# FelixWaiblinger/gym-pybullet-adrp

Measured on AMD Instinct MI355X. Metric: env-steps/sec (N parallel drones) at 1/2/4/8 MI355X; % HBM roofline, higher is better.
Workload: dtype f64; 1 GPU; HoverAviary Physics.PYB 240/30 Hz (8 sub-steps), 4096 envs x 1 drone per GPU, RPM actions, auto-reset; envs_per_gpu=4096, global_envs=4096, drones_per_env=1, parallelism=env-sharded dp1

## Files before the change

### gym_pybullet_adrp_amd/csrc/adrp_device.h

```cpp
#pragma once

#include <hip/hip_runtime.h>
#include <stdint.h>

namespace adrp {

__device__ __forceinline__ void store_out(float4* p, float4 v) {
#ifdef ADRP_NT_STORES
    typedef float f4v __attribute__((ext_vector_type(4)));
    const f4v w = {v.x, v.y, v.z, v.w};
    __builtin_nontemporal_store(w, reinterpret_cast<f4v*>(p));
#else
    *p = v;
#endif
}

#ifdef ADRP_RACE_TIMING
__device__ unsigned long long g_race_phase[32];
#define RACE_MARK(var) const uint64_t var = __builtin_amdgcn_s_memtime()
#define RACE_SET(var) var = __builtin_amdgcn_s_memtime()
#define RACE_ACC(i, dt) do { atomicAdd(&g_race_phase[i], (unsigned long long)(dt)); \
        atomicMax(&g_race_phase[10 + (i)], (unsigned long long)(dt)); } while (0)
constexpr int kWaveSlots = 16384;
__device__ unsigned long long g_race_wave[kWaveSlots * 8];
// ... 367 lines not shown
    if (x < 0.0f) r = 3.14159265358979323846f - r;
    return copysignf(r, y);
}
__device__ __forceinline__ double fatan2_(double y, double x) { return f64::atan2(y, x); }
__device__ __forceinline__ float fatan2_nc_(float y, float x) { return fatan2_(y, x); }
__device__ __forceinline__ double fatan2_nc_(double y, double x) { return f64::atan2_nc(y, x); }
__device__ __forceinline__ float fasin_(float s) { return fatan2_(s, __builtin_amdgcn_sqrtf((1.0f - s) * (1.0f + s))); }
__device__ __forceinline__ double fasin_(double s) { return f64::asin(s); }
__device__ __forceinline__ float fexp_(float x) { return __builtin_amdgcn_exp2f(x * 1.4426950408889634f); }
__device__ __forceinline__ double fexp_(double x) { return f64::exp(x); }

template <typename Real>
struct ChainK {
    Real k004, c100, nn_min, near1, tiny;
    Real ts[3], tc[4];
};
template <typename Real>
__device__ __forceinline__ ChainK<Real> chain_consts() {
    return ChainK<Real>{Real(0.04), Real(100), Real(1e-300), Real(1e-9), Real(0.03),
                        {Real(-0.0001984126984126984), Real(0.008333333333333333), Real(-0.16666666666666666)},
                        {Real(2.48015873015873e-05), Real(-0.001388888888888889), Real(0.041666666666666664), Real(-0.5)}};
}
__device__ __forceinline__ void pin(double& x) { asm volatile("" : "+v"(x)); }
__device__ __forceinline__ void pin(float&) {}
template <typename Real>
__device__ __forceinline__ void pin_all(ChainK<Real>& k) {
    pin(k.k004); pin(k.c100); pin(k.nn_min); pin(k.near1); pin(k.tiny);
#pragma unroll
    for (int i = 0; i < 3; ++i) pin(k.ts[i]);
#pragma unroll
    for (int i = 0; i < 4; ++i) pin(k.tc[i]);
}
__device__ __forceinline__ float hsqrt_nn_(float x, const ChainK<float>&) { return __builtin_amdgcn_sqrtf(x); }
__device__ __forceinline__ double hsqrt_nn_(double x, const ChainK<double>& k) {
    const double y = __builtin_amdgcn_rsq(__builtin_fmax(x, k.nn_min));
    double g = x * y, h = 0.5 * y;
#pragma unroll
    for (int i = 0; i < 2; ++i) {
        const double r = f64::fma_(-g, h, 0.5);
        g = f64::fma_(g, r, g);
        h = f64::fma_(h, r, h);
    }
    const double d = f64::fma_(-g, g, x);
    return f64::fma_(d, h, g);
}
__device__ __forceinline__ void expmap_sinc_cos(float x, float* sinc, float* c, const ChainK<float>&) {
    expmap_sinc_cos(x, sinc, c);
}
__device__ __forceinline__ void expmap_sinc_cos(double x, double* sinc, double* c, const ChainK<double>& k) {
    const double x2 = x * x;
    const bool tiny = __builtin_fabs(x) <= k.tiny;
    double ps = f64::fma_(k.ts[0], x2, k.ts[1]);
    ps = f64::fma_(ps, x2, k.ts[2]);
    double pc = f64::fma_(k.tc[0], x2, k.tc[1]);
    pc = f64::fma_(pc, x2, k.tc[2]);
    pc = f64::fma_(pc, x2, k.tc[3]);
    if (__builtin_expect(!__all(tiny), 0)) {
        double fs, fc;
        expmap_sinc_cos_full(x, &fs, &fc);
        *sinc = tiny ? f64::fma_(x2, ps, 1.0) : fs;
        *c = tiny ? f64::fma_(x2, pc, 1.0) : fc;
        return;
    }
    *sinc = f64::fma_(x2, ps, 1.0);
    *c = f64::fma_(x2, pc, 1.0);
}
struct AngK {
    double p[10];
    double tan8, pi4, pi2, pi;
    double lim, lo, hi;
};
__device__ __forceinline__ AngK ang_consts() {
    return AngK{{0.021428368220326288, -0.04375458729368037, 0.05699267039194693, -0.06642647883966969,
                 0.07690277001250925, -0.09090800003785938, 0.11111107550967636, -0.14285714221246087,
                 0.19999999999459742, -0.3333333333333199},
                0.41421356237309504880, 0.78539816339744830962, 1.57079632679489661923, 3.14159265358979323846,
                0.99999, 1e-150, 1e150};
}
__device__ __forceinline__ void pin_all(AngK& k) {
#pragma unroll
    for (int i = 0; i < 10; ++i) pin(k.p[i]);
    pin(k.tan8); pin(k.pi4); pin(k.pi2); pin(k.pi); pin(k.lim); pin(k.lo); pin(k.hi);
}
namespace f64 {
__device__ __forceinline__ bool atan2_lean_ok(double y, double x, const AngK& k) {
    const double s = __builtin_fabs(x) + __builtin_fabs(y);
    return s > k.lo && s < k.hi;
}
template <bool XPOS>
__device__ __forceinline__ double atan2_lean(double y, double x, const AngK& k) {
    const double ax = __builtin_fabs(x), ay = __builtin_fabs(y);
    const double mx = __builtin_fmax(ax, ay), mn = __builtin_fmin(ax, ay);
    const bool big = mn > k.tan8 * mx;
    const double num = big ? mn - mx : mn, den = big ? mn + mx : mx;
    const double t = num * rcp_nc(den);
    const double s = t * t;
    double p = k.p[0];
#pragma unroll
    for (int i = 1; i < 10; ++i) p = fma_(p, s, k.p[i]);
    double r = fma_(t * s, p, t);
    if (big) r += k.pi4;
    if (ay > ax) r = k.pi2 - r;
    if constexpr (!XPOS) {
        if (x < 0.0) r = k.pi - r;
    }
    return __builtin_copysign(r, y);
}
__device__ __forceinline__ double asin_lean(double s, const AngK& k) {
    const double x = (1.0 - s) * (1.0 + s);
    const double y = __builtin_amdgcn_rsq(x);
    double g = x * y, h = 0.5 * y;
#pragma unroll
    for (int i = 0; i < 2; ++i) {
        const double r = fma_(-g, h, 0.5);
        g = fma_(g, r, g);
        h = fma_(h, r, h);
    }
    const double d = fma_(-g, g, x);
    return atan2_lean<true>(s, fma_(d, h, g), k);
}
}

__device__ __forceinline__ float quat_inv_norm(float n2, const ChainK<float>&) { return quat_inv_norm(n2); }
__device__ __forceinline__ double quat_inv_norm(double n2, const ChainK<double>& k) {
    const bool near1 = __builtin_fabs(n2 - 1.0) <= k.near1;
    const double newton = f64::fma_(0.5, 1.0 - n2, 1.0);
    if (__builtin_expect(__all(near1), 1)) return newton;
    const double r = f64::rsq_nc(n2);
    return near1 ? newton : r;
}

__device__ __forceinline__ void clamp100_wv(V3<float>& w, V3<float>& v) {
    w = {__builtin_amdgcn_fmed3f(w.x, -100.0f, 100.0f), __builtin_amdgcn_fmed3f(w.y, -100.0f, 100.0f),
         __builtin_amdgcn_fmed3f(w.z, -100.0f, 100.0f)};
    v = {__builtin_amdgcn_fmed3f(v.x, -100.0f, 100.0f), __builtin_amdgcn_fmed3f(v.y, -100.0f, 100.0f),
         __builtin_amdgcn_fmed3f(v.z, -100.0f, 100.0f)};
}
__device__ __forceinline__ double clamp100_sel(double x) { return x < -100.0 ? -100.0 : (x > 100.0 ? 100.0 : x); }
__device__ __forceinline__ void clamp100_wv(V3<double>& w, V3<double>& v) {
    const bool big = (__builtin_fabs(w.x) > 100.0) | (__builtin_fabs(w.y) > 100.0) | (__builtin_fabs(w.z) > 100.0) |
                     (__builtin_fabs(v.x) > 100.0) | (__builtin_fabs(v.y) > 100.0) | (__builtin_fabs(v.z) > 100.0);
    if (__builtin_expect(__any(big), 0)) {
        w = {clamp100_sel(w.x), clamp100_sel(w.y), clamp100_sel(w.z)};
        v = {clamp100_sel(v.x), clamp100_sel(v.y), clamp100_sel(v.z)};
    }
}


template <typename Real>
__device__ __forceinline__ M3<Real> rot(Q4<Real> q) {
    const Real x2 = q.x + q.x, y2 = q.y + q.y, z2 = q.z + q.z;
    const Real xx = q.x * x2, yy = q.y * y2, zz = q.z * z2;
    const Real xy = q.x * y2, xz = q.x * z2, yz = q.y * z2;
    const Real wx = q.w * x2, wy = q.w * y2, wz = q.w * z2;
    return {Real(1) - (yy + zz), xy - wz, xz + wy,
            xy + wz, Real(1) - (xx + zz), yz - wx,
            xz - wy, yz + wx, Real(1) - (xx + yy)};
}
template <typename Real>
__device__ __forceinline__ V3<Real> mul(const M3<Real>& R, V3<Real> v) {
    return {R.a00 * v.x + R.a01 * v.y + R.a02 * v.z,
            R.a10 * v.x + R.a11 * v.y + R.a12 * v.z,
            R.a20 * v.x + R.a21 * v.y + R.a22 * v.z};
}
template <typename Real>
__device__ __forceinline__ V3<Real> mulT(const M3<Real>& R, V3<Real> v) {
// ... 154 lines not shown
```

### gym_pybullet_adrp_amd/csrc/hover_kernel.h

```cpp
#pragma once

#include "adrp_device.h"
#include "dslpid_core.h"

namespace adrp {

enum HoverField {
    HF_POS = 0, HF_QUAT = 3, HF_VEL = 7, HF_OMEGA = 10, HF_LAST_RPM = 13, HF_ANGV = 17,
    HF_LINK_QUAT = 20, HF_NBASE = 24,
    HF_PID = 24, HF_NPID = 9
};
enum HoverInt { HI_STEP = 0, HI_EPISODE = 1, HI_RING_HEAD = 2, HI_N = 3 };

template <typename Real>
struct HoverConst {
    int S, trunc_steps, link_lag, physics;
    Real dt, mass, inv_mass, gravity;
    Real ixx, iyy, izz, inv_ixx, inv_iyy, inv_izz;
    Real kf, km, hover_rpm;
    Real px[4], py[4], pz[4];
    Real gnd_kf, prop_r4, gnd_clip;
    Real drag[3];
    Real dyn_arm;
    Real coll_hh, coll_r, coll_zoff;
// ... 297 lines not shown
               c * q.z + k * (w.y * q.x - w.x * q.y + w.z * q.w),
               c * q.w + k * (-w.x * q.x - w.y * q.y - w.z * q.z)};
    }
    b.angv = mul(R, b.w);
}

template <typename Real>
__device__ __forceinline__ void hover_reset_draw(const HoverReset<Real>& a, uint64_t seed, uint64_t gid, uint32_t tag,
                                                 const HoverConst<Real>& C, Body<Real>& b, int32_t& sc, int32_t& ep) {
    const U4 r0 = draw(seed, gid, uint32_t(ep), tag, 0);
    const U4 r1 = draw(seed, gid, uint32_t(ep), tag, 1);
    const U4 r2 = draw(seed, gid, uint32_t(ep), tag, 2);
    const uint32_t w0[4] = {r0.a, r0.b, r0.c, r0.d}, w1[4] = {r1.a, r1.b, r1.c, r1.d},
                   w2[4] = {r2.a, r2.b, r2.c, r2.d};
    Real p[3], e_[3], v[3], om[3];
#pragma unroll
    for (int k = 0; k < 3; ++k) {
        p[k] = a.init_xyz[k] + a.n_xyz[k] * (Real(2) * u01r<Real>(w0[k]) - Real(1));
        e_[k] = a.init_rpy[k] + a.n_rpy[k] * (Real(2) * u01r<Real>(w1[k]) - Real(1));
        v[k] = a.n_vel[k] * (Real(2) * u01r<Real>(w2[k]) - Real(1));
    }
    om[0] = a.n_om[0] * (Real(2) * u01r<Real>(w0[3]) - Real(1));
    om[1] = a.n_om[1] * (Real(2) * u01r<Real>(w1[3]) - Real(1));
    om[2] = a.n_om[2] * (Real(2) * u01r<Real>(w2[3]) - Real(1));
    b.q = quat_from_euler_fast<Real>(e_[0], e_[1], e_[2]);
    b.pos = v3(p[0], p[1], p[2]);
    b.ql = b.q;
    b.vel = v3(v[0], v[1], v[2]);
    if (C.physics == ADRP_PHYS_DYN) {
        b.w = mulT(rot(b.q), v3(om[0], om[1], om[2]));
        b.angv = v3(om[0], om[1], om[2]);
    } else {
        b.w = v3(om[0], om[1], om[2]);
        b.angv = v3(Real(0), Real(0), Real(0));
    }
#pragma unroll
    for (int i = 0; i < 4; ++i) b.prev_rpm[i] = Real(0);
    sc = 0;
    ep += 1;
}
template <typename Real>
__device__ __forceinline__ void hover_reset_state(const HoverArgs<Real>& args, const HoverConst<Real>& C, int e,
                                                  Body<Real>& b, int32_t& sc, int32_t& ep) {
    hover_reset_draw(*args.r, args.seed, uint64_t(args.env_offset + e), TAG_HOVER_RESET, C, b, sc, ep);
}

template <typename Real>
__device__ __forceinline__ Real euler_roll_u(Q4<Real> q) {
    if (__builtin_expect(__any(fabs_(euler_sarg(q)) >= Real(0.99999)), 0)) return euler_xyz_fast(q).x;
    const EulerArgs<Real> a = euler_args(q);
    return fatan2_(a.y0, a.x0);
}
template <typename Real>
__device__ __forceinline__ Real euler_pitch_u(Q4<Real> q) {
    const Real sarg = euler_sarg(q);
    if (__builtin_expect(__any(fabs_(sarg) >= Real(0.99999)), 0)) return euler_xyz_fast(q).y;
    return fasin_(sarg);
}
template <typename Real>
__device__ __forceinline__ Real euler_yaw_u(Q4<Real> q) {
    if (__builtin_expect(__any(fabs_(euler_sarg(q)) >= Real(0.99999)), 0)) return euler_xyz_fast(q).z;
    const EulerArgs<Real> a = euler_args(q);
    return fatan2_(a.y2, a.x2);
}

__device__ __forceinline__ double euler_roll_lean(Q4<double> q, const AngK& k) {
    const EulerArgs<double> a = euler_args(q);
    const bool ok = fabs_(a.sarg) < k.lim && f64::atan2_lean_ok(a.y0, a.x0, k);
    if (__builtin_expect(__any(!ok), 0)) return euler_roll_u(q);
    return f64::atan2_lean<false>(a.y0, a.x0, k);
}
__device__ __forceinline__ double euler_pitch_lean(Q4<double> q, const AngK& k) {
    const double sarg = euler_sarg(q);
    if (__builtin_expect(__any(!(fabs_(sarg) < k.lim)), 0)) return euler_pitch_u(q);
    return f64::asin_lean(sarg, k);
}
__device__ __forceinline__ double euler_yaw_lean(Q4<double> q, const AngK& k) {
    const EulerArgs<double> a = euler_args(q);
    const bool ok = fabs_(a.sarg) < k.lim && f64::atan2_lean_ok(a.y2, a.x2, k);
    if (__builtin_expect(__any(!ok), 0)) return euler_yaw_u(q);
    return f64::atan2_lean<false>(a.y2, a.x2, k);
}

template <typename Real>
__device__ __forceinline__ Real euler_axis_u(Q4<Real> q, int ax) {
    const EulerArgs<Real> a = euler_args(q);
    const Real sarg = a.sarg;
    if (__builtin_expect(__any(fabs_(sarg) >= Real(0.99999)), 0)) {
        const V3<Real> r = euler_xyz_fast(q);
        return ax == 0 ? r.x : (ax == 1 ? r.y : r.z);
    }
    const Real y0 = a.y0, x0 = a.x0, y2 = a.y2, x2 = a.x2;
    Real x1;
    if constexpr (sizeof(Real) == 8) x1 = f64::sqrt((1.0 - sarg) * (1.0 + sarg));
    else x1 = __builtin_amdgcn_sqrtf((1.0f - sarg) * (1.0f + sarg));
    const Real yy = ax == 0 ? y0 : (ax == 1 ? sarg : y2), xx = ax == 0 ? x0 : (ax == 1 ? x1 : x2);
    return fatan2_(yy, xx);
}
__device__ __forceinline__ float readlane_r(float v, int l) {
    return __int_as_float(__builtin_amdgcn_readlane(__float_as_int(v), l));
}
__device__ __forceinline__ double readlane_r(double v, int l) {
    return __hiloint2double(__builtin_amdgcn_readlane(__double2hiint(v), l), __builtin_amdgcn_readlane(__double2loint(v), l));
}
template <typename Real>
__device__ __forceinline__ V3<Real> hover_obs12_split(const HoverConst<Real>& a, const Body<Real>& b, float o[12]) {
    const int l = int(threadIdx.x) & 63;
    const Real ang = euler_axis_u(b.q, l < 2 ? l : 2);
    const V3<Real> rpy = v3(readlane_r(ang, 0), readlane_r(ang, 1), readlane_r(ang, 2));
    const V3<Real> w = a.physics == ADRP_PHYS_DYN ? b.angv : b.w;
    o[0] = float(b.pos.x); o[1] = float(b.pos.y); o[2] = float(b.pos.z);
    o[3] = float(rpy.x);   o[4] = float(rpy.y);   o[5] = float(rpy.z);
    o[6] = float(b.vel.x); o[7] = float(b.vel.y); o[8] = float(b.vel.z);
    o[9] = float(w.x);     o[10] = float(w.y);    o[11] = float(w.z);
    return rpy;
}

template <typename Real>
__device__ __forceinline__ V3<Real> hover_obs12(const HoverConst<Real>& a, const Body<Real>& b, float o[12]) {
    const V3<Real> rpy = euler_xyz_fast_u(b.q);
    const V3<Real> w = a.physics == ADRP_PHYS_DYN ? b.angv : b.w;
    o[0] = float(b.pos.x); o[1] = float(b.pos.y); o[2] = float(b.pos.z);
    o[3] = float(rpy.x);   o[4] = float(rpy.y);   o[5] = float(rpy.z);
    o[6] = float(b.vel.x); o[7] = float(b.vel.y); o[8] = float(b.vel.z);
    o[9] = float(w.x);     o[10] = float(w.y);    o[11] = float(w.z);
    return rpy;
}

template <int A, int B>
__device__ __forceinline__ void write_row(float* row, const float o12[12], const float (&ring)[B][A], int head1) {
    if constexpr (A == 4) {
        float4* r4 = reinterpret_cast<float4*>(row);
        r4[0] = make_float4(o12[0], o12[1], o12[2], o12[3]);
        r4[1] = make_float4(o12[4], o12[5], o12[6], o12[7]);
        r4[2] = make_float4(o12[8], o12[9], o12[10], o12[11]);
#pragma unroll
        for (int p = 0; p < B; ++p) {
            int k = p - head1;
            k += k < 0 ? B : 0;
            r4[3 + k] = make_float4(ring[p][0], ring[p][1], ring[p][2], ring[p][3]);
        }
    } else {
#pragma unroll
        for (int k = 0; k < 12; ++k) row[k] = o12[k];
#pragma unroll
        for (int p = 0; p < B; ++p) {
            int k = p - head1;
            k += k < 0 ? B : 0;
#pragma unroll
            for (int j = 0; j < A; ++j) row[12 + k * A + j] = ring[p][j];
        }
    }
}

template <int A>
__device__ __forceinline__ void write_row_generic(float* __restrict__ row, const float o12[12],
                                                  const float* __restrict__ ring, int B, int E, int e, int head1,
                                                  const float act[A], bool act_is_newest) {
#pragma unroll
    for (int k = 0; k < 12; ++k) row[k] = o12[k];
    constexpr int CH = 8;
    int slot = head1;
    for (int k0 = 0; k0 < B; k0 += CH) {
        float v[CH][A];
#pragma unroll
        for (int c = 0; c < CH; ++c) {
// ... 197 lines not shown
struct NoExtForce {};
template <typename Real, int PH, int SC, bool DRAG, typename Ext>
__device__ __forceinline__ bool pyb_chain(const HoverConst<Real>& C, Body<Real>& b, const Real rpm_in[4], bool lag,
                                          Ext ext, V3<Real>* wb_out = nullptr, Real* vxy = nullptr) {
    constexpr bool EXT = !__is_same(Ext, NoExtForce);
    const Real rpm[4] = {rpm_in[0], rpm_in[1], rpm_in[2], rpm_in[3]};
    Real sum_f = 0, t2 = 0;
    V3<Real> P = v3(Real(0), Real(0), Real(0));
#pragma unroll
    for (int i = 0; i < 4; ++i) {
        const Real r2 = rpm[i] * rpm[i];
        const Real f = r2 * C.kf;
        sum_f += f;
        const bool pz0 = __builtin_constant_p(C.pz[i]) && C.pz[i] == Real(0);
        const Real fx = f * C.px[i], fy = f * C.py[i], fz = f * C.pz[i];
        P = v3(P.x + fx, P.y + fy, pz0 ? P.z : P.z + fz);
        t2 += (i & 1) ? -r2 : r2;
    }
    const Real tau_z = t2 * C.km;
    ChainK<Real> K = chain_consts<Real>();
    HoverConst<Real> Cp = C;
    if constexpr (sizeof(Real) == 8) {
        pin_all(K);
        pin(Cp.dt); pin(Cp.mass); pin(Cp.gravity); pin(Cp.inv_mass); pin(Cp.ang_max);
        pin(Cp.ixx); pin(Cp.iyy); pin(Cp.izz); pin(Cp.inv_ixx); pin(Cp.inv_iyy); pin(Cp.inv_izz);
        pin(Cp.coll_hh); pin(Cp.coll_r); pin(Cp.coll_zoff);
    }
    Chain<Real> st{};
    {
        const M3<Real> R = rot_fm(b.q);
        const M3<Real> Rs = lag ? rot_fm(b.ql) : R;
        st.wb = mulT(R, b.w);
        st.zc = col2(R);
        st.zs = col2(Rs);
        st.m3 = lag ? mulT(R, st.zs) : v3(Real(0), Real(0), Real(1));
        if constexpr (DRAG) {
            st.R = R;
            st.Rs = Rs;
        }
    }
    st.wn = hsqrt_nn_(dot(b.w, b.w), K);
    st.dti = v3(Cp.dt * Cp.inv_ixx, Cp.dt * Cp.inv_iyy, Cp.dt * Cp.inv_izz);
    bool touched = false;
    auto substep = [&](int s) {
        if constexpr (EXT) touched |= pyb_substep<Real, PH, true>(Cp, b, st, rpm, sum_f, P, tau_z, K, ext(b, st));
        else touched |= pyb_substep<Real, PH>(Cp, b, st, rpm, sum_f, P, tau_z, K, V3<Real>{}, vxy ? vxy + 2 * s : nullptr);
#pragma unroll
        for (int i = 0; i < 4; ++i) b.prev_rpm[i] = rpm[i];
    };
    if constexpr (SC > 0) {
#pragma unroll
        for (int s = 0; s < SC; ++s) substep(s);
    } else {
        for (int s = 0; s < C.S; ++s) substep(s);
    }
    if (wb_out) *wb_out = st.wb;
    else b.w = mul(rot_fm(b.q), st.wb);
    return touched;
}

constexpr int kRowF4 = 18;

template <int A, int B>
__device__ __forceinline__ void stage_row(float4* lds_row, const float o12[12], const float (&ring)[B][A], int head1) {
    lds_row[0] = make_float4(o12[0], o12[1], o12[2], o12[3]);
    lds_row[1] = make_float4(o12[4], o12[5], o12[6], o12[7]);
    lds_row[2] = make_float4(o12[8], o12[9], o12[10], o12[11]);
#pragma unroll
    for (int p = 0; p < B; ++p) {
        int k = p - head1;
        k += k < 0 ? B : 0;
        lds_row[3 + k] = make_float4(ring[p][0], ring[p][1], ring[p][2], ring[p][3]);
    }
}

template <typename Real, int PH, int A, int B, int SC, bool STG = false, int CTL = 0, bool HELP = false, int SYS = 0,
          int FO = 2>
__device__ __forceinline__ void hover_step_body(const HoverArgs<Real>& a, const HoverConst<Real>& C,
                                                const float* pre = nullptr) {
    constexpr int BR = B > 0 ? B : 1;
    constexpr bool DRAG = (PH == ADRP_PHYS_PYB_DRAG || PH == ADRP_PHYS_PYB_GND_DRAG_DW);
    constexpr bool DYN = (PH == ADRP_PHYS_DYN);
    static_assert(!HELP || STG, "the reset helper wave pairs with the staged (all lanes live) kernel");
    __shared__ Real rs_body[HELP ? kResetFields * kStepBlock : 1];
    __shared__ float rs_obs[HELP ? 12 * kStepBlock : 1];
    __shared__ float4 rows[STG ? kStepBlock * kRowF4 : 1];
    constexpr bool ANG = HELP && angle_helpers<Real>();
    __shared__ Real ang_q[ANG ? 4 * kStepBlock : 1];
    __shared__ Real ang_r[ANG ? kStepBlock : 1];
    __shared__ Real ang_p[ANG ? kStepBlock : 1];
    __shared__ float ang_y[ANG ? kStepBlock : 1];
    constexpr int kWaves = HELP ? 1 + help_waves<Real>() : 1;
    constexpr auto cb = [](int w) { return w == 0 ? 0 : (w >= kWaves ? kRowF4 : (kWaves == 2 ? kRowF4 / 2 : 5 * w - 2)); };
    constexpr bool TROWS = ANG;
    constexpr int kSplitCols = 5, kSplitRows = 12;
    static_assert(!TROWS || (cb(2) - cb(1) == kSplitCols && cb(4) - cb(3) == kSplitCols && cb(1) == 3 &&
                             kSplitCols * kSplitRows <= kStepBlock), "terminal rows: 3 + 3 x 5 columns");
    __shared__ int done_cnt[1];
    __shared__ uint8_t done_list[TROWS ? kStepBlock : 1];
    [[maybe_unused]] auto helper_tail = [&](int tl, int wv) {
        const int cnt_v = done_cnt[0];
        const int sub = tl / kSplitCols, c = cb(wv) + tl - kSplitCols * sub;
        const int row0 = done_list[sub] & (kStepBlock - 1);
        float4* dst = reinterpret_cast<float4*>(a.obs) + size_t(blockIdx.x) * kStepBlock * kRowF4;
        float4 o[kSplitCols];
#pragma unroll
        for (int j = 0; j < kSplitCols; ++j) o[j] = rows[tl + kStepBlock * (cb(wv) + j)];
        const float4 t0 = rows[row0 * kRowF4 + c];
#pragma unroll
        for (int j = 0; j < kSplitCols; ++j) store_out(dst + tl + kStepBlock * (cb(wv) + j), o[j]);
        const int cnt = __builtin_amdgcn_readfirstlane(cnt_v);
        const bool mine = tl < kSplitCols * kSplitRows;
        float4* tb = reinterpret_cast<float4*>(a.tobs) + size_t(blockIdx.x) * kStepBlock * kRowF4;
        if (mine && sub < cnt) tb[row0 * kRowF4 + c] = t0;
        for (int base = kSplitRows; base < cnt && base < kStepBlock; base += kSplitRows) {
            const int n = base + sub;
            if (mine && n < cnt) {
                const int row = done_list[n] & (kStepBlock - 1);
                tb[row * kRowF4 + c] = rows[row * kRowF4 + c];
            }
        }
    };
    if constexpr (HELP) {
        if (ANG && threadIdx.x >= 2 * kStepBlock) {
            const int tl = threadIdx.x & (kStepBlock - 1), wv = threadIdx.x / kStepBlock;
            AngK ak = ang_consts();
            pin_all(ak);
            __syncthreads();
            const Q4<Real> q = {ang_q[tl], ang_q[kStepBlock + tl], ang_q[2 * kStepBlock + tl], ang_q[3 * kStepBlock + tl]};
            if constexpr (ANG) {
                if (wv == 2) ang_p[tl] = euler_pitch_lean(q, ak);
                else ang_y[tl] = float(euler_yaw_lean(q, ak));
            }
            __syncthreads();
            __syncthreads();
            if constexpr (TROWS) {
                helper_tail(tl, wv);
                return;
            }
            float4* dst = reinterpret_cast<float4*>(a.obs) + size_t(blockIdx.x) * kStepBlock * kRowF4;
            for (int k = cb(wv); k < cb(wv + 1); ++k) store_out(dst + tl + kStepBlock * k, rows[tl + kStepBlock * k]);
            return;
        }
        if (threadIdx.x >= kStepBlock) {
            const int tl = threadIdx.x - kStepBlock;
            const int he = blockIdx.x * kStepBlock + tl;
            const int E = a.E;
            const float4 av = reinterpret_cast<const float4*>(a.act)[he];
            float rg[BR][4];
#pragma unroll
            for (int p = 0; p < B; ++p) {
                const float4 v = reinterpret_cast<const float4*>(a.ring)[size_t(p) * E + he];
                rg[p][0] = v.x; rg[p][1] = v.y; rg[p][2] = v.z; rg[p][3] = v.w;
            }
            const int32_t head = a.ist[HI_RING_HEAD * E + he];
            int32_t hsc = 0, hep = a.ist[HI_EPISODE * E + he];
            Body<Real> rb;
            hover_reset_state(a, C, he, rb, hsc, hep);
            float o[12];
            hover_obs12(C, rb, o);
            const Real v[kResetFields] = {rb.pos.x, rb.pos.y, rb.pos.z, rb.q.x, rb.q.y, rb.q.z, rb.q.w,
                                          rb.vel.x, rb.vel.y, rb.vel.z, rb.w.x, rb.w.y, rb.w.z,
                                          rb.angv.x, rb.angv.y, rb.angv.z};
#pragma unroll
            for (int k = 0; k < kResetFields; ++k) rs_body[k * kStepBlock + tl] = v[k];
#pragma unroll
            for (int k = 0; k < 12; ++k) rs_obs[k * kStepBlock + tl] = o[k];
            float4* my = rows + tl * kRowF4;
            const int hu = __builtin_amdgcn_readfirstlane(head);
            if (__all(head == hu)) {
                const int h1 = hu + 1 == B ? 0 : hu + 1;
#pragma unroll
                for (int p = 0; p < B; ++p) {
                    const int k = p >= h1 ? p - h1 : p - h1 + B;
                    my[3 + k] = make_float4(rg[p][0], rg[p][1], rg[p][2], rg[p][3]);
                }
                my[3 + B - 1] = av;
            } else {
                const int h1 = head + 1 == B ? 0 : head + 1;
#pragma unroll
                for (int p = 0; p < B; ++p) {
                    int k = p - h1;
                    k += k < 0 ? B : 0;
                    const bool hit = p == head;
                    my[3 + k] = make_float4(hit ? av.x : rg[p][0], hit ? av.y : rg[p][1], hit ? av.z : rg[p][2],
                                            hit ? av.w : rg[p][3]);
                }
            }
            reinterpret_cast<float4*>(a.ring)[size_t(head) * E + he] = av;
            [[maybe_unused]] AngK ak = ang_consts();
            if constexpr (ANG) pin_all(ak);
            __syncthreads();
            if constexpr (ANG) {
                const Q4<Real> q = {ang_q[tl], ang_q[kStepBlock + tl], ang_q[2 * kStepBlock + tl], ang_q[3 * kStepBlock + tl]};
                ang_r[tl] = euler_roll_lean(q, ak);
                __syncthreads();
            }
            __syncthreads();
            if constexpr (TROWS) {
                helper_tail(tl, 1);
                return;
            }
            float4* dst = reinterpret_cast<float4*>(a.obs) + size_t(blockIdx.x) * kStepBlock * kRowF4;
#pragma unroll
            for (int k = cb(1); k < cb(2); ++k) store_out(dst + tl + kStepBlock * k, rows[tl + kStepBlock * k]);
            return;
        }
    }
    const int E = a.E;
    const bool split = ADRP_PERSIST_SPLIT && !STG && !HELP && E == 1;
    const int e = split ? 0 : int(blockIdx.x) * kStepBlock + int(threadIdx.x);
    const int D = B > 0 ? 12 + B * A : a.D;
    if (e >= E) return;
    RACE_MARK(t0);
    const bool fit = FO == 2 ? field_offsets_fit<Real>(E) : FO == 1;
    const bool lag = C.link_lag && !DYN;
    const BodyOffs<Real> fo = body_offsets<Real>(E, e, lag, DRAG, DYN);
    uint32_t io[HI_N];
    field_run(uint32_t(e) * 4u, uint32_t(E) * 4u, 0, HI_N, io);
    Body<Real> b;
    int32_t sc, ep, head_ld;
    if (fit) {
        load_body_at<Real>(a.f, fo, b, lag, DRAG, DYN);
        sc = field_at(a.ist, io[HI_STEP]); ep = field_at(a.ist, io[HI_EPISODE]); head_ld = field_at(a.ist, io[HI_RING_HEAD]);
        field_form_end();
    } else {
        load_body(a, e, b, lag, DRAG, DYN);
        sc = a.ist[HI_STEP * E + e]; ep = a.ist[HI_EPISODE * E + e]; head_ld = a.ist[HI_RING_HEAD * E + e];
    }
    const int32_t head = head_ld;
    float act[A];
    if constexpr (SYS == 2) {
#pragma unroll
        for (int j = 0; j < A; ++j) act[j] = pre[j];
    } else if constexpr (SYS == 1) {
        uint32_t* sa = const_cast<uint32_t*>(reinterpret_cast<const uint32_t*>(a.act)) + size_t(e) * A;
#pragma unroll
        for (int j = 0; j < A; ++j)
            act[j] = __uint_as_float(__hip_atomic_load(sa + j, __ATOMIC_RELAXED, __HIP_MEMORY_SCOPE_SYSTEM));
    } else if constexpr (A == 4) {
        const float4 v = reinterpret_cast<const float4*>(a.act)[e];
        act[0] = v.x; act[1] = v.y; act[2] = v.z; act[3] = v.w;
    } else {
#pragma unroll
        for (int j = 0; j < A; ++j) act[j] = a.act[e * A + j];
    }
    float ring[BR][A];
#pragma unroll
    for (int p = 0; p < (HELP ? 0 : B); ++p) {
        if constexpr (A == 4) {
            const float4 v = reinterpret_cast<const float4*>(a.ring)[size_t(p) * E + e];
            ring[p][0] = v.x; ring[p][1] = v.y; ring[p][2] = v.z; ring[p][3] = v.w;
        } else {
#pragma unroll
            for (int j = 0; j < A; ++j) ring[p][j] = a.ring[(size_t(p) * E + e) * A + j];
        }
    }
    Real rpm[4];
    if constexpr (CTL != 0) {
        static_assert(A == (CTL == ADRP_ACT_PID ? 3 : CTL == ADRP_ACT_VEL ? 4 : 1), "PID action width");
        Real ctl[HF_NPID];
        uint32_t po[HF_PID + HF_NPID];
        field_run(uint32_t(e) * uint32_t(sizeof(Real)), uint32_t(E) * uint32_t(sizeof(Real)), HF_PID, HF_NPID, po);
        if (fit) {
#pragma unroll
            for (int k = 0; k < HF_NPID; ++k) ctl[k] = field_at(a.f, po[HF_PID + k]);
            field_form_end();
        } else {
#pragma unroll
            for (int k = 0; k < HF_NPID; ++k) ctl[k] = a.f[(HF_PID + k) * E + e];
        }
        dslpid_rpm<Real, CTL>(C, b, act, ctl, rpm);
        if (fit) {
#pragma unroll
            for (int k = 0; k < HF_NPID; ++k) field_last(a.f, po[HF_PID + k]) = ctl[k];
            field_form_end();
        } else {
#pragma unroll
            for (int k = 0; k < HF_NPID; ++k) a.f[(HF_PID + k) * E + e] = ctl[k];
        }
    } else {
#pragma unroll
        for (int i = 0; i < 4; ++i) rpm[i] = C.hover_rpm * Real(rpm_gain(act[A == 1 ? 0 : i]));
    }
    bool touched = false;
    V3<Real> wbf = v3(Real(0), Real(0), Real(0));
    constexpr bool LATE_XY = ANG && !DYN && SC > 0;
    Real vxy[LATE_XY ? 2 * SC : 2] = {};
#ifdef ADRP_RACE_TIMING
    __builtin_amdgcn_s_waitcnt(0);
#endif
    RACE_MARK(t1);
    if constexpr (DYN) {
        if constexpr (SC > 0) {
#pragma unroll
            for (int s = 0; s < SC; ++s) dyn_substep(C, b, rpm);
        } else {
            for (int s = 0; s < C.S; ++s) dyn_substep(C, b, rpm);
        }
    } else {
        touched = pyb_chain<Real, PH, SC, DRAG>(C, b, rpm, lag, NoExtForce{}, ANG ? &wbf : nullptr, LATE_XY ? vxy : nullptr);
    }
    RACE_MARK(t2);
    if (touched && a.contact_count && (!split || threadIdx.x == 0)) atomicAdd(a.contact_count, 1);
    if constexpr (HELP) {
    } else if constexpr (A == 4)
        reinterpret_cast<float4*>(a.ring)[size_t(head) * E + e] = make_float4(act[0], act[1], act[2], act[3]);
    else
#pragma unroll
        for (int j = 0; j < A; ++j) a.ring[(size_t(head) * E + e) * A + j] = act[j];
    const int BB = B > 0 ? B : a.B;
    const int head1 = head + 1 == BB ? 0 : head + 1;
    auto store_state = [&]() {
        if (fit) {
            store_body_at<Real>(a.f, fo, b, lag, DRAG, DYN);
            field_last(a.ist, io[HI_STEP]) = sc;
            field_last(a.ist, io[HI_EPISODE]) = ep;
            field_last(a.ist, io[HI_RING_HEAD]) = head1;
            field_form_end();
        } else {
            store_body(a, e, b, lag, DRAG, DYN);
            a.ist[HI_STEP * E + e] = sc;
            a.ist[HI_EPISODE * E + e] = ep;
            a.ist[HI_RING_HEAD * E + e] = head1;
        }
    };
    float o12[12];
    V3<Real> rpy;
    if constexpr (ANG) {
        const int tl = threadIdx.x;
        ang_q[tl] = b.q.x; ang_q[kStepBlock + tl] = b.q.y; ang_q[2 * kStepBlock + tl] = b.q.z;
        ang_q[3 * kStepBlock + tl] = b.q.w;
        __syncthreads();
        hold(b.q.x); hold(b.q.y); hold(b.q.z); hold(b.q.w);
        hold(wbf.x); hold(wbf.y); hold(wbf.z);
        hold(b.pos.x); hold(b.pos.y); hold(b.pos.z);
        if constexpr (LATE_XY) {
#pragma unroll
            for (int k = 0; k < 2 * SC; ++k) hold(vxy[k]);
#pragma unroll
            for (int s = 0; s < SC; ++s) {
                b.pos.x = fmx(C.dt, vxy[2 * s], b.pos.x);
                b.pos.y = fmx(C.dt, vxy[2 * s + 1], b.pos.y);
            }
        }
        hold(b.vel.x); hold(b.vel.y); hold(b.vel.z);
        if constexpr (!DYN) b.w = mul(rot_fm(b.q), wbf);
        const V3<Real> w = C.physics == ADRP_PHYS_DYN ? b.angv : b.w;
        o12[0] = float(b.pos.x); o12[1] = float(b.pos.y); o12[2] = float(b.pos.z);
        o12[6] = float(b.vel.x); o12[7] = float(b.vel.y); o12[8] = float(b.vel.z);
        o12[9] = float(w.x);     o12[10] = float(w.y);    o12[11] = float(w.z);
    } else if (split) {
        rpy = hover_obs12_split(C, b, o12);
    } else {
        rpy = hover_obs12(C, b, o12);
    }
    const Real dx = C.target[0] - b.pos.x, dy = C.target[1] - b.pos.y, dz = C.target[2] - b.pos.z;
    const Real d2 = dx * dx + dy * dy + dz * dz;
    const Real r = Real(2) - d2 * d2;
    a.rew[e] = float(r > Real(0) ? r : Real(0));
    const bool te = d2 < Real(1e-8);
    bool tr = fabs_(b.pos.x) > Real(1.5) || fabs_(b.pos.y) > Real(1.5) || b.pos.z > Real(2.0) || sc >= C.trunc_steps;
    if constexpr (ANG) {
        hold(b.w.x); hold(b.w.y); hold(b.w.z);
#pragma unroll
        for (int k = 0; k < 12; ++k)
            if (k < 3 || k > 5) hold(o12[k]);
        __syncthreads();
        rpy.x = ang_r[threadIdx.x];
        rpy.y = ang_p[threadIdx.x];
        o12[3] = float(rpy.x);
        o12[4] = float(rpy.y);
        o12[5] = ang_y[threadIdx.x];
    }
    tr = tr || fabs_(rpy.x) > Real(0.4) || fabs_(rpy.y) > Real(0.4);
    a.term[e] = te;
    a.trunc[e] = tr;
    sc += C.S;
    const bool done = a.autoreset && (te || tr);
    RACE_MARK(t3);
#ifdef ADRP_RACE_TIMING
    const unsigned long long dmask = __ballot(done);
    uint64_t t4 = 0;
#endif
    if constexpr (STG) {
        static_assert(A == 4 && B == 15, "staged rows: 72-float rows only");
        float4* my = rows + threadIdx.x * kRowF4;
        const int hu = __builtin_amdgcn_readfirstlane(head);
        if constexpr (HELP) {
        } else if (__all(head == hu)) {
            const int h1 = hu + 1 == B ? 0 : hu + 1;
#pragma unroll
            for (int p = 0; p < B; ++p) {
                const int k = p >= h1 ? p - h1 : p - h1 + B;
                my[3 + k] = make_float4(ring[p][0], ring[p][1], ring[p][2], ring[p][3]);
            }
            my[3 + B - 1] = make_float4(act[0], act[1], act[2], act[3]);
        } else {
#pragma unroll
            for (int p = 0; p < B; ++p) {
                const bool hit = p == head;
#pragma unroll
                for (int j = 0; j < A; ++j) ring[p][j] = hit ? act[j] : ring[p][j];
            }
            stage_row<A, B>(my, o12, ring, head1);
        }
        my[0] = make_float4(o12[0], o12[1], o12[2], o12[3]);
        my[1] = make_float4(o12[4], o12[5], o12[6], o12[7]);
        my[2] = make_float4(o12[8], o12[9], o12[10], o12[11]);
        if constexpr (HELP && !ANG) __syncthreads();
        if constexpr (TROWS) {
            const unsigned long long done_mask = __ballot(done);
            done_cnt[0] = a.tobs ? __popcll(done_mask) : 0;
            if (done && a.tobs) {
                float4* trow = reinterpret_cast<float4*>(a.tobs + size_t(e) * D);
                trow[0] = make_float4(o12[0], o12[1], o12[2], o12[3]);
                trow[1] = make_float4(o12[4], o12[5], o12[6], o12[7]);
                trow[2] = make_float4(o12[8], o12[9], o12[10], o12[11]);
                const uint32_t rank = __builtin_amdgcn_mbcnt_hi(uint32_t(done_mask >> 32), __builtin_amdgcn_mbcnt_lo(uint32_t(done_mask), 0u));
                done_list[rank] = uint8_t(threadIdx.x);
            }
        }
        if (done) {
            if (!TROWS && a.tobs) {
                float4 t[kRowF4];
#pragma unroll
                for (int k = 0; k < kRowF4; ++k) t[k] = my[k];
                float4* trow = reinterpret_cast<float4*>(a.tobs + size_t(e) * D);
#pragma unroll
                for (int k = 0; k < kRowF4; ++k) trow[k] = t[k];
            }
            if constexpr (HELP) {
                const int t = threadIdx.x;
                Real v[kResetFields];
#pragma unroll
                for (int k = 0; k < kResetFields; ++k) v[k] = rs_body[k * kStepBlock + t];
                b.pos = v3(v[0], v[1], v[2]);
                b.q = {v[3], v[4], v[5], v[6]};
                b.ql = b.q;
                b.vel = v3(v[7], v[8], v[9]);
                b.w = v3(v[10], v[11], v[12]);
                b.angv = v3(v[13], v[14], v[15]);
#pragma unroll
                for (int i = 0; i < 4; ++i) b.prev_rpm[i] = Real(0);
                sc = 0;
                ep += 1;
#pragma unroll
                for (int k = 0; k < 12; ++k) o12[k] = rs_obs[k * kStepBlock + t];
            } else {
                hover_reset_state(a, C, e, b, sc, ep);
                hover_obs12(C, b, o12);
            }
            my[0] = make_float4(o12[0], o12[1], o12[2], o12[3]);
            my[1] = make_float4(o12[4], o12[5], o12[6], o12[7]);
            my[2] = make_float4(o12[8], o12[9], o12[10], o12[11]);
        }
        RACE_SET(t4);
        store_state();
        __syncthreads();
        float4* dst = reinterpret_cast<float4*>(a.obs) + size_t(blockIdx.x) * kStepBlock * kRowF4;
        constexpr int KC = cb(1);
#pragma unroll
        for (int k = 0; k < KC; ++k) store_out(dst + threadIdx.x + kStepBlock * k, rows[threadIdx.x + kStepBlock * k]);
    } else {
#pragma unroll
        for (int p = 0; p < B; ++p) {
            const bool hit = p == head;
#pragma unroll
            for (int j = 0; j < A; ++j) ring[p][j] = hit ? act[j] : ring[p][j];
        }
        if (done) {
            if (a.tobs) {
                if constexpr (B > 0) write_row<A, B>(a.tobs + size_t(e) * D, o12, ring, head1);
                else write_row_generic<A>(a.tobs + size_t(e) * D, o12, a.ring, a.B, E, e, head1, act, true);
            }
            hover_reset_state(a, C, e, b, sc, ep);
            if (split) hover_obs12_split(C, b, o12);
            else hover_obs12(C, b, o12);
        }
        RACE_SET(t4);
        if constexpr (B > 0) write_row<A, B>(a.obs + size_t(e) * D, o12, ring, head1);
        else write_row_generic<A>(a.obs + size_t(e) * D, o12, a.ring, a.B, E, e, head1, act, true);
    }
    RACE_MARK(t5);
    if constexpr (!STG) {
        store_state();
    }
#ifdef ADRP_RACE_TIMING
    RACE_MARK(t6);
    if (threadIdx.x == 0) {
        RACE_ACC(0, t1 - t0); RACE_ACC(1, t2 - t1); RACE_ACC(2, t3 - t2); RACE_ACC(3, t4 - t3);
        RACE_ACC(4, t5 - t4); RACE_ACC(5, t6 - t5); RACE_ACC(6, t6 - t0); RACE_ACC(8, 1);
        RACE_ACC(7, __popcll(dmask));
        if (dmask) atomicAdd(&g_race_phase[9], 1ull);
    }
#endif
}

template <typename Real>
struct HoverTail {
    const HoverConst<Real>* c;
    const HoverReset<Real>* r;
    uint8_t* term;
    uint8_t* trunc;
    float* tobs;
    int32_t* contact_count;
    uint64_t seed;
    int64_t env_offset;
    int B, D, autoreset;
};

template <typename Real, int PH, int A, int B, bool DEF, bool STG = false, int CTL = 0, bool HELP = false, bool W32 = true>
__global__ void __launch_bounds__(256) hover_step_kernel(Real* f, float* ring, int32_t* ist, const float* act,
                                                         float* obs, float* rew, int E, HoverTail<Real> t) {
    HoverArgs<Real> a;
    a.c = t.c; a.r = t.r;
    a.f = f; a.ring = ring; a.ist = ist; a.act = act; a.obs = obs; a.rew = rew;
    a.term = t.term; a.trunc = t.trunc; a.tobs = t.tobs; a.mask = nullptr; a.contact_count = t.contact_count;
    a.seed = t.seed; a.env_offset = t.env_offset;
    a.E = E; a.B = t.B; a.D = t.D; a.autoreset = t.autoreset;
    if constexpr (DEF) {
        constexpr HoverConst<Real> C = cf2x_consts<Real>(PH);
        hover_step_body<Real, PH, A, B, C.S, STG, CTL, HELP, 0, W32 ? 1 : 0>(a, C);
    } else {
        hover_step_body<Real, PH, A, B, 0, STG, CTL, HELP, 0, W32 ? 1 : 0>(a, *a.c);
    }
}

template <typename Real, int A>
__global__ void __launch_bounds__(256) hover_reset_kernel(HoverArgs<Real> a) {
    const int e = blockIdx.x * blockDim.x + threadIdx.x;
    if (e >= a.E || (a.mask && !a.mask[e])) return;
    const HoverConst<Real>& C = *a.c;
    const int E = a.E;
    const bool dyn = C.physics == ADRP_PHYS_DYN;
    const bool drag = C.physics == ADRP_PHYS_PYB_DRAG || C.physics == ADRP_PHYS_PYB_GND_DRAG_DW;
    Body<Real> b;
    int32_t sc = a.ist[HI_STEP * E + e], ep = a.ist[HI_EPISODE * E + e];
    const int head = a.ist[HI_RING_HEAD * E + e];
    hover_reset_state(a, C, e, b, sc, ep);
    store_body(a, e, b, C.link_lag && !dyn, drag, dyn);
    a.ist[HI_STEP * E + e] = sc;
    a.ist[HI_EPISODE * E + e] = ep;
    float o12[12];
    hover_obs12(C, b, o12);
    const float none[A] = {};
// ... 5 lines not shown
```

Baseline: 765.8 million env-steps/s.

## Decide truncation from quaternion directly and move obs copy-out to helper waves

```diff
diff --git a/gym_pybullet_adrp_amd/csrc/adrp_device.h b/gym_pybullet_adrp_amd/csrc/adrp_device.h
--- a/gym_pybullet_adrp_amd/csrc/adrp_device.h
+++ b/gym_pybullet_adrp_amd/csrc/adrp_device.h
@@ -473,6 +473,20 @@
     for (int i = 0; i < 10; ++i) pin(k.p[i]);
     pin(k.tan8); pin(k.pi4); pin(k.pi2); pin(k.pi); pin(k.lim); pin(k.lo); pin(k.hi);
 }
+constexpr double kTruncBand = 1e-9;
+struct TruncK {
+    double s_lo, s_hi, t_lo, t_hi;
+    double lim;
+};
+__device__ __forceinline__ TruncK trunc_consts() {
+    return TruncK{0.3894183423086505 * (1.0 - kTruncBand), 0.3894183423086505 * (1.0 + kTruncBand),
+                  0.4227932187381618 * (1.0 - kTruncBand), 0.4227932187381618 * (1.0 + kTruncBand), 0.99999};
+}
+__device__ __forceinline__ void pin_s(double& x) { asm volatile("" : "+s"(x)); }
+__device__ __forceinline__ void pin_all(TruncK& k) {
+    pin_s(k.s_lo); pin_s(k.s_hi); pin_s(k.t_lo); pin_s(k.t_hi); pin_s(k.lim);
+}
+
 namespace f64 {
 __device__ __forceinline__ bool atan2_lean_ok(double y, double x, const AngK& k) {
     const double s = __builtin_fabs(x) + __builtin_fabs(y);
diff --git a/gym_pybullet_adrp_amd/csrc/hover_kernel.h b/gym_pybullet_adrp_amd/csrc/hover_kernel.h
--- a/gym_pybullet_adrp_amd/csrc/hover_kernel.h
+++ b/gym_pybullet_adrp_amd/csrc/hover_kernel.h
@@ -403,6 +403,16 @@
     return f64::atan2_lean<false>(a.y2, a.x2, k);
 }
 
+__device__ __forceinline__ bool trunc_from_quat(Q4<double> q, const TruncK& k, bool& over) {
+    const EulerArgs<double> a = euler_args(q);
+    const double as = fabs_(a.sarg), ay = fabs_(a.y0);
+    const bool p_over = as > k.s_hi, r_over = ay > k.t_hi * a.x0;
+    const bool p_sure = p_over || as < k.s_lo, r_sure = r_over || ay < k.t_lo * a.x0;
+    over = p_over || r_over;
+    return p_sure && r_sure && a.x0 > 0.0 && as < k.lim;
+}
+__device__ __forceinline__ bool trunc_from_quat(Q4<float>, const TruncK&, bool&) { return false; }
+
 template <typename Real>
 __device__ __forceinline__ Real euler_axis_u(Q4<Real> q, int ax) {
     const EulerArgs<Real> a = euler_args(q);
@@ -766,38 +776,72 @@
     constexpr bool DRAG = (PH == ADRP_PHYS_PYB_DRAG || PH == ADRP_PHYS_PYB_GND_DRAG_DW);
     constexpr bool DYN = (PH == ADRP_PHYS_DYN);
     static_assert(!HELP || STG, "the reset helper wave pairs with the staged (all lanes live) kernel");
+    constexpr bool ANG = HELP && angle_helpers<Real>();
     __shared__ Real rs_body[HELP ? kResetFields * kStepBlock : 1];
-    __shared__ float rs_obs[HELP ? 12 * kStepBlock : 1];
-    __shared__ float4 rows[STG ? kStepBlock * kRowF4 : 1];
-    constexpr bool ANG = HELP && angle_helpers<Real>();
+    __shared__ float rs_obs[HELP && !ANG ? 12 * kStepBlock : 1];
+    constexpr int kResetObs = kStepBlock * kRowF4;
+    __shared__ float4 rows[STG ? kStepBlock * kRowF4 + (ANG ? 3 * kStepBlock : 0) : 1];
     __shared__ Real ang_q[ANG ? 4 * kStepBlock : 1];
     __shared__ Real ang_r[ANG ? kStepBlock : 1];
     __shared__ Real ang_p[ANG ? kStepBlock : 1];
     __shared__ float ang_y[ANG ? kStepBlock : 1];
     constexpr int kWaves = HELP ? 1 + help_waves<Real>() : 1;
-    constexpr auto cb = [](int w) { return w == 0 ? 0 : (w >= kWaves ? kRowF4 : (kWaves == 2 ? kRowF4 / 2 : 5 * w - 2)); };
+    constexpr auto cb = [](int w) { return w == 0 ? 0 : (w >= kWaves ? kRowF4 : (kWaves == 2 ? kRowF4 / 2 : 6 * (w - 1))); };
     constexpr bool TROWS = ANG;
-    constexpr int kSplitCols = 5, kSplitRows = 12;
-    static_assert(!TROWS || (cb(2) - cb(1) == kSplitCols && cb(4) - cb(3) == kSplitCols && cb(1) == 3 &&
-                             kSplitCols * kSplitRows <= kStepBlock), "terminal rows: 3 + 3 x 5 columns");
+    constexpr int kHelpLanes = 3 * kStepBlock, kRingF4 = kRowF4 - 3;
+    constexpr int kRingPer = kStepBlock * kRingF4 / kHelpLanes;
+    constexpr int kTermRows = kHelpLanes / kRowF4;
+    static_assert(!TROWS || (kWaves == 4 && kRingPer * kHelpLanes == kStepBlock * kRingF4 && cb(1) == 0),
+                  "copy-out over three helper waves");
     __shared__ int done_cnt[1];
     __shared__ uint8_t done_list[TROWS ? kStepBlock : 1];
-    [[maybe_unused]] auto helper_tail = [&](int tl, int wv) {
+    __shared__ uint8_t done_b[TROWS ? kStepBlock : 1];
+    struct TailIdx {
+        uint32_t ring[kRingPer], kin, fix, flag, sub, tcol;
+    };
+    [[maybe_unused]] auto tail_index = [&](int tl, int wv) {
+        TailIdx t;
+        const uint32_t g = uint32_t(wv - 1) * kStepBlock + uint32_t(tl);
+#pragma unroll
+        for (int j = 0; j < kRingPer; ++j) {
+            const uint32_t n = g + kHelpLanes * uint32_t(j);
+            const uint32_t row = (n * 4370u) >> 16;
+            t.ring[j] = (row * kRowF4 + 3u + (n - kRingF4 * row)) * 16u;
+            asm volatile("" : "+v"(t.ring[j]));
+        }
+        t.flag = (g * 21846u) >> 16;
+        t.kin = (t.flag * kRowF4 + (g - 3u * t.flag)) * 16u;
+        t.fix = (kResetObs + g) * 16u;
+        t.sub = (g * 3641u) >> 16;
+        t.tcol = g - kRowF4 * t.sub;
+        asm volatile("" : "+v"(t.kin), "+v"(t.fix), "+v"(t.flag), "+v"(t.sub), "+v"(t.tcol));
+        return t;
+    };
+    [[maybe_unused]] auto helper_ring = [&](const TailIdx& ti) {
+        const char* lds = reinterpret_cast<const char*>(rows);
+        char* dst = reinterpret_cast<char*>(a.obs) + size_t(blockIdx.x) * (kStepBlock * kRowF4 * sizeof(float4));
+        float4 o[kRingPer];
+#pragma unroll
+        for (int j = 0; j < kRingPer; ++j) o[j] = *reinterpret_cast<const float4*>(lds + ti.ring[j]);
+#pragma unroll
+        for (int j = 0; j < kRingPer; ++j) store_out(reinterpret_cast<float4*>(dst + ti.ring[j]), o[j]);
+    };
+    [[maybe_unused]] auto helper_tail = [&](const TailIdx& ti) {
         const int cnt_v = done_cnt[0];
-        const int sub = tl / kSplitCols, c = cb(wv) + tl - kSplitCols * sub;
-        const int row0 = done_list[sub] & (kStepBlock - 1);
-        float4* dst = reinterpret_cast<float4*>(a.obs) + size_t(blockIdx.x) * kStepBlock * kRowF4;
-        float4 o[kSplitCols];
-#pragma unroll
-        for (int j = 0; j < kSplitCols; ++j) o[j] = rows[tl + kStepBlock * (cb(wv) + j)];
-        const float4 t0 = rows[row0 * kRowF4 + c];
-#pragma unroll
-        for (int j = 0; j < kSplitCols; ++j) store_out(dst + tl + kStepBlock * (cb(wv) + j), o[j]);
+        const int row0 = done_list[ti.sub] & (kStepBlock - 1);
+        const uint8_t fl = done_b[ti.flag];
+        const char* lds = reinterpret_cast<const char*>(rows);
+        char* dst = reinterpret_cast<char*>(a.obs) + size_t(blockIdx.x) * (kStepBlock * kRowF4 * sizeof(float4));
+        const float4 o = *reinterpret_cast<const float4*>(lds + (fl ? ti.fix : ti.kin));
+        float4 t0 = rows[row0 * kRowF4 + int(ti.tcol)];
+        hold(t0.x); hold(t0.y); hold(t0.z); hold(t0.w);
+        store_out(reinterpret_cast<float4*>(dst + ti.kin), o);
         const int cnt = __builtin_amdgcn_readfirstlane(cnt_v);
-        const bool mine = tl < kSplitCols * kSplitRows;
+        const int sub = int(ti.sub), c = int(ti.tcol);
+        const bool mine = sub < kTermRows;
         float4* tb = reinterpret_cast<float4*>(a.tobs) + size_t(blockIdx.x) * kStepBlock * kRowF4;
         if (mine && sub < cnt) tb[row0 * kRowF4 + c] = t0;
-        for (int base = kSplitRows; base < cnt && base < kStepBlock; base += kSplitRows) {
+        for (int base = kTermRows; base < cnt && base < kStepBlock; base += kTermRows) {
             const int n = base + sub;
             if (mine && n < cnt) {
                 const int row = done_list[n] & (kStepBlock - 1);
@@ -810,16 +854,26 @@
             const int tl = threadIdx.x & (kStepBlock - 1), wv = threadIdx.x / kStepBlock;
             AngK ak = ang_consts();
             pin_all(ak);
+            const TailIdx ti = tail_index(tl, wv);
             __syncthreads();
             const Q4<Real> q = {ang_q[tl], ang_q[kStepBlock + tl], ang_q[2 * kStepBlock + tl], ang_q[3 * kStepBlock + tl]};
             if constexpr (ANG) {
-                if (wv == 2) ang_p[tl] = euler_pitch_lean(q, ak);
-                else ang_y[tl] = float(euler_yaw_lean(q, ak));
-            }
+                float* rowf = reinterpret_cast<float*>(rows) + tl * (4 * kRowF4);
+                if (wv == 2) {
+                    const double p = euler_pitch_lean(q, ak);
+                    ang_p[tl] = p;
+                    rowf[4] = float(p);
+                } else {
+                    const float y = float(euler_yaw_lean(q, ak));
+                    ang_y[tl] = y;
+                    rowf[5] = y;
+                }
+            }
+            if constexpr (TROWS) helper_ring(ti);
             __syncthreads();
             __syncthreads();
             if constexpr (TROWS) {
-                helper_tail(tl, wv);
+                helper_tail(ti);
                 return;
             }
             float4* dst = reinterpret_cast<float4*>(a.obs) + size_t(blockIdx.x) * kStepBlock * kRowF4;
@@ -848,8 +902,14 @@
                                           rb.angv.x, rb.angv.y, rb.angv.z};
 #pragma unroll
             for (int k = 0; k < kResetFields; ++k) rs_body[k * kStepBlock + tl] = v[k];
-#pragma unroll
-            for (int k = 0; k < 12; ++k) rs_obs[k * kStepBlock + tl] = o[k];
+            if constexpr (ANG) {
+                rows[kResetObs + 3 * tl + 0] = make_float4(o[0], o[1], o[2], o[3]);
+                rows[kResetObs + 3 * tl + 1] = make_float4(o[4], o[5], o[6], o[7]);
+                rows[kResetObs + 3 * tl + 2] = make_float4(o[8], o[9], o[10], o[11]);
+            } else {
+#pragma unroll
+                for (int k = 0; k < 12; ++k) rs_obs[k * kStepBlock + tl] = o[k];
+            }
             float4* my = rows + tl * kRowF4;
             const int hu = __builtin_amdgcn_readfirstlane(head);
             if (__all(head == hu)) {
@@ -874,15 +934,20 @@
             reinterpret_cast<float4*>(a.ring)[size_t(head) * E + he] = av;
             [[maybe_unused]] AngK ak = ang_consts();
             if constexpr (ANG) pin_all(ak);
+            [[maybe_unused]] TailIdx ti{};
+            if constexpr (TROWS) ti = tail_index(tl, 1);
             __syncthreads();
             if constexpr (ANG) {
                 const Q4<Real> q = {ang_q[tl], ang_q[kStepBlock + tl], ang_q[2 * kStepBlock + tl], ang_q[3 * kStepBlock + tl]};
-                ang_r[tl] = euler_roll_lean(q, ak);
+                const double roll = euler_roll_lean(q, ak);
+                ang_r[tl] = roll;
+                reinterpret_cast<float*>(rows)[tl * (4 * kRowF4) + 3] = float(roll);
+                if constexpr (TROWS) helper_ring(ti);
                 __syncthreads();
             }
             __syncthreads();
             if constexpr (TROWS) {
-                helper_tail(tl, 1);
+                helper_tail(ti);
                 return;
             }
             float4* dst = reinterpret_cast<float4*>(a.obs) + size_t(blockIdx.x) * kStepBlock * kRowF4;
@@ -1045,19 +1110,27 @@
     a.rew[e] = float(r > Real(0) ? r : Real(0));
     const bool te = d2 < Real(1e-8);
     bool tr = fabs_(b.pos.x) > Real(1.5) || fabs_(b.pos.y) > Real(1.5) || b.pos.z > Real(2.0) || sc >= C.trunc_steps;
+    [[maybe_unused]] bool slow = false;
     if constexpr (ANG) {
         hold(b.w.x); hold(b.w.y); hold(b.w.z);
 #pragma unroll
         for (int k = 0; k < 12; ++k)
             if (k < 3 || k > 5) hold(o12[k]);
-        __syncthreads();
-        rpy.x = ang_r[threadIdx.x];
-        rpy.y = ang_p[threadIdx.x];
-        o12[3] = float(rpy.x);
-        o12[4] = float(rpy.y);
-        o12[5] = ang_y[threadIdx.x];
-    }
-    tr = tr || fabs_(rpy.x) > Real(0.4) || fabs_(rpy.y) > Real(0.4);
+        TruncK tk = trunc_consts();
+        pin_all(tk);
+        bool over = false;
+        const bool sure = trunc_from_quat(b.q, tk, over);
+        slow = __any(!sure);
+        if (__builtin_expect(slow, 0)) {
+            __syncthreads();
+            rpy.x = ang_r[threadIdx.x];
+            rpy.y = ang_p[threadIdx.x];
+            over = fabs_(rpy.x) > Real(0.4) || fabs_(rpy.y) > Real(0.4);
+        }
+        tr = tr || over;
+    } else {
+        tr = tr || fabs_(rpy.x) > Real(0.4) || fabs_(rpy.y) > Real(0.4);
+    }
     a.term[e] = te;
     a.trunc[e] = tr;
     sc += C.S;
@@ -1089,32 +1162,17 @@
             }
             stage_row<A, B>(my, o12, ring, head1);
         }
-        my[0] = make_float4(o12[0], o12[1], o12[2], o12[3]);
-        my[1] = make_float4(o12[4], o12[5], o12[6], o12[7]);
-        my[2] = make_float4(o12[8], o12[9], o12[10], o12[11]);
-        if constexpr (HELP && !ANG) __syncthreads();
         if constexpr (TROWS) {
+            float* mf = reinterpret_cast<float*>(my);
+            mf[0] = o12[0]; mf[1] = o12[1]; mf[2] = o12[2];
+            mf[6] = o12[6]; mf[7] = o12[7];
+            my[2] = make_float4(o12[8], o12[9], o12[10], o12[11]);
             const unsigned long long done_mask = __ballot(done);
+            done_b[threadIdx.x] = done;
             done_cnt[0] = a.tobs ? __popcll(done_mask) : 0;
-            if (done && a.tobs) {
-                float4* trow = reinterpret_cast<float4*>(a.tobs + size_t(e) * D);
-                trow[0] = make_float4(o12[0], o12[1], o12[2], o12[3]);
-                trow[1] = make_float4(o12[4], o12[5], o12[6], o12[7]);
-                trow[2] = make_float4(o12[8], o12[9], o12[10], o12[11]);
+            if (done) {
                 const uint32_t rank = __builtin_amdgcn_mbcnt_hi(uint32_t(done_mask >> 32), __builtin_amdgcn_mbcnt_lo(uint32_t(done_mask), 0u));
                 done_list[rank] = uint8_t(threadIdx.x);
-            }
-        }
-        if (done) {
-            if (!TROWS && a.tobs) {
-                float4 t[kRowF4];
-#pragma unroll
-                for (int k = 0; k < kRowF4; ++k) t[k] = my[k];
-                float4* trow = reinterpret_cast<float4*>(a.tobs + size_t(e) * D);
-#pragma unroll
-                for (int k = 0; k < kRowF4; ++k) trow[k] = t[k];
-            }
-            if constexpr (HELP) {
                 const int t = threadIdx.x;
                 Real v[kResetFields];
 #pragma unroll
@@ -1129,23 +1187,58 @@
                 for (int i = 0; i < 4; ++i) b.prev_rpm[i] = Real(0);
                 sc = 0;
                 ep += 1;
-#pragma unroll
-                for (int k = 0; k < 12; ++k) o12[k] = rs_obs[k * kStepBlock + t];
-            } else {
-                hover_reset_state(a, C, e, b, sc, ep);
-                hover_obs12(C, b, o12);
-            }
+            }
+            RACE_SET(t4);
+            store_state();
+            if (!slow) __syncthreads();
+            __syncthreads();
+        } else {
             my[0] = make_float4(o12[0], o12[1], o12[2], o12[3]);
             my[1] = make_float4(o12[4], o12[5], o12[6], o12[7]);
             my[2] = make_float4(o12[8], o12[9], o12[10], o12[11]);
-        }
-        RACE_SET(t4);
-        store_state();
-        __syncthreads();
-        float4* dst = reinterpret_cast<float4*>(a.obs) + size_t(blockIdx.x) * kStepBlock * kRowF4;
-        constexpr int KC = cb(1);
-#pragma unroll
-        for (int k = 0; k < KC; ++k) store_out(dst + threadIdx.x + kStepBlock * k, rows[threadIdx.x + kStepBlock * k]);
+            if constexpr (HELP) __syncthreads();
+            if (done) {
+                if (a.tobs) {
+                    float4 t[kRowF4];
+#pragma unroll
+                    for (int k = 0; k < kRowF4; ++k) t[k] = my[k];
+                    float4* trow = reinterpret_cast<float4*>(a.tobs + size_t(e) * D);
+#pragma unroll
+                    for (int k = 0; k < kRowF4; ++k) trow[k] = t[k];
+                }
+                if constexpr (HELP) {
+                    const int t = threadIdx.x;
+                    Real v[kResetFields];
+#pragma unroll
+                    for (int k = 0; k < kResetFields; ++k) v[k] = rs_body[k * kStepBlock + t];
+                    b.pos = v3(v[0], v[1], v[2]);
+                    b.q = {v[3], v[4], v[5], v[6]};
+                    b.ql = b.q;
+                    b.vel = v3(v[7], v[8], v[9]);
+                    b.w = v3(v[10], v[11], v[12]);
+                    b.angv = v3(v[13], v[14], v[15]);
+#pragma unroll
+                    for (int i = 0; i < 4; ++i) b.prev_rpm[i] = Real(0);
+                    sc = 0;
+                    ep += 1;
+#pragma unroll
+                    for (int k = 0; k < 12; ++k) o12[k] = rs_obs[k * kStepBlock + t];
+                } else {
+                    hover_reset_state(a, C, e, b, sc, ep);
+                    hover_obs12(C, b, o12);
+                }
+                my[0] = make_float4(o12[0], o12[1], o12[2], o12[3]);
+                my[1] = make_float4(o12[4], o12[5], o12[6], o12[7]);
+                my[2] = make_float4(o12[8], o12[9], o12[10], o12[11]);
+            }
+            RACE_SET(t4);
+            store_state();
+            __syncthreads();
+            float4* dst = reinterpret_cast<float4*>(a.obs) + size_t(blockIdx.x) * kStepBlock * kRowF4;
+            constexpr int KC = cb(1);
+#pragma unroll
+            for (int k = 0; k < KC; ++k) store_out(dst + threadIdx.x + kStepBlock * k, rows[threadIdx.x + kStepBlock * k]);
+        }
     } else {
 #pragma unroll
         for (int p = 0; p < B; ++p) {
```

After: 793.3 million env-steps/s, median of 6. +3.6%, better.
